# pg42819/EscTp1RayTracer

Measured on AMD Instinct MI355X. Metric: Mrays/sec + frame ms, 3840x2160 / 10k spheres, at 1/2/4/8 MI355X, higher is better.
Workload: dtype f32

## Files before the change

esctp1raytracer_amd/__init__.py:

```python
import ctypes as C

import numpy as np

from . import _capi
from ._capi import (ESC_FACE_FIXED, ESC_FACE_HASH, ESC_STAGE_AUTO, ESC_STAGE_BVH, ESC_STAGE_LDS,
                    ESC_RENDER_EXACT_ONLY, ESC_RENDER_INDEX_ORDER, ESC_RENDER_SHADE_FUSED,
                    ESC_RENDER_SHADE_QUEUE, ESC_RENDER_TIME_KERNELS, ESC_RENDER_NO_TILE_LISTS, ESC_RENDER_NO_LIGHT_LISTS, ESC_RENDER_TWO_KERNELS, ESC_RENDER_BVH_HEURISTIC_PADS, ESC_RENDER_NO_COUNTERS, ESC_RENDER_NO_PACKED_LIGHT_LISTS, ESC_RENDER_VOTE,
                    ESC_STAGE_SMEM, ESC_TRANSMIT_OFF, ESC_TRANSMIT_REFRACT, ESC_TRANSMIT_FRESNEL, EscError,
                    check)

__all__ = ["Scene", "Camera", "Renderer", "RecordedFrame", "TemporalAccumulator", "FlatScene", "MultiRenderer", "render_multi", "render_multi_rccl", "rccl_available", "strip_local_rows", "live_device_allocations", "trace", "write_ppm", "quantise", "synthetic_view", "ambient_table", "environment_sky", "environment_lookup_host",
           "EscError", "ESC_FACE_FIXED", "ESC_FACE_HASH", "ESC_STAGE_AUTO", "ESC_STAGE_SMEM",
           "ESC_STAGE_LDS", "ESC_STAGE_BVH", "ESC_RENDER_EXACT_ONLY", "ESC_RENDER_TIME_KERNELS", "ESC_RENDER_INDEX_ORDER", "ESC_RENDER_SHADE_QUEUE",
           "ESC_RENDER_SHADE_FUSED", "ESC_RENDER_NO_TILE_LISTS", "ESC_RENDER_NO_LIGHT_LISTS", "ESC_RENDER_TWO_KERNELS", "ESC_RENDER_BVH_HEURISTIC_PADS", "ESC_RENDER_NO_COUNTERS", "ESC_RENDER_NO_PACKED_LIGHT_LISTS", "ESC_RENDER_VOTE", "ESC_TRANSMIT_OFF", "ESC_TRANSMIT_REFRACT", "ESC_TRANSMIT_FRESNEL", "version"]


def _f32(a, shape=None):
    a = np.ascontiguousarray(a, dtype=np.float32)
    if shape is not None:
        a = a.reshape(shape)
    return a


def _fp(a):
# ... 970 lines not shown
                "cap": hdr[5], "global_cap": hdr[6], "counts": cnt.reshape(hdr[4], hdr[3])}

    def tile_list_ids(self, which, index):
        hdr = (C.c_int32 * 8)()
        if check(self._lib.esc_tile_list_counts(self._h, which, hdr, None, 0)) == 0:
            return np.zeros(0, np.int32), 0
        cap = hdr[6] if index < 0 else hdr[5]
        ids = np.zeros(cap, np.int32)
        n = check(self._lib.esc_tile_list_ids(self._h, which, int(index),
                                              ids.ctypes.data_as(C.POINTER(C.c_int32)), cap))
        return ids[:min(n, cap)].copy(), n

    def tile_list_global(self, which):
        return self.tile_list_ids(which, -1)

    def light_lists(self, which):
        info = (C.c_int32 * 8)()
        i32 = C.POINTER(C.c_int32)
        n = check(self._lib.esc_light_list_read(self._h, which, info, None, None, 0, 0, None))
        if n == 0:
            return None
        n_listed, R, cap, gcap = info[0], info[1], info[2], info[3]
        per_light = 6 * R * R
        face_counts = np.zeros((n_listed, 6), np.int32)
        face_ids = np.zeros((n_listed, 6, gcap), np.int32)
        ids = np.zeros((n_listed, 6, R, R, cap), np.int32)
        for li in range(n_listed):
            check(self._lib.esc_light_list_read(self._h, which, info, face_counts.ctypes.data_as(i32),
                                                face_ids.ctypes.data_as(i32), li * per_light, per_light,
                                                ids[li].ctypes.data_as(i32)))
# ... 203 lines not shown
```

esctp1raytracer_amd/_capi.py:

```python
import ctypes as C
import os

_HERE = os.path.dirname(os.path.abspath(__file__))
LIB_PATH = os.environ.get("ESC_LIB_PATH") or os.path.join(_HERE, "lib", "libesctp1rt.so")

ESC_OK = 0
ESC_ERR_INVALID = -1
ESC_ERR_HIP = -2
ESC_ERR_IO = -3
ESC_ERR_PARSE = -4
ESC_ERR_NOMEM = -5
ESC_ERR_NO_DEVICE = -6
ESC_ERR_RCCL = -7

ESC_FACE_FIXED = 0
ESC_FACE_HASH = 1
ESC_STAGE_AUTO = 0
ESC_STAGE_SMEM = 1
ESC_STAGE_LDS = 2
ESC_STAGE_BVH = 3
ESC_MATERIAL_FLOATS = 13
ESC_TRANSMISSION_FLOATS = 4
ESC_TRANSMIT_OFF = 0
ESC_TRANSMIT_REFRACT = 1
# ... 210 lines not shown
    "esc_frame_destroy": (None, [_P]),
    "esc_strip_local_rows": (C.c_int, [C.c_int32, C.c_int32, C.c_int32, C.c_int32]),
    "esc_assemble_strips": (C.c_int, [_P, _P, C.c_int32, C.c_size_t, C.c_int32, C.c_int32,
                                      C.c_int32, C.c_int32, _P]),
    "esc_build_accel": (C.c_int, [_P, _F]),
    "esc_get_accel_info": (C.c_int, [_P, C.POINTER(esc_accel_info)]),
    "esc_scene_build_accel": (C.c_int, [_P, _F, C.c_int32, C.POINTER(esc_accel_info),
                                        C.POINTER(esc_bvh_node), C.c_int64, _I32, C.c_int64, _F,
                                        C.c_int64]),
    "esc_scene_table": (C.c_int64, [_P, C.c_int32, _P, C.c_int64]),
    "esc_queue_schedule": (C.c_int, [C.c_int32, C.c_int32, _I32, C.c_int32]),
    "esc_tri_group_record": (C.c_int, [_F, C.c_int32, _F]),
    "esc_sphere_group_record": (C.c_int, [_F, C.c_int32, _F]),
    "esc_tile_list_counts": (C.c_int, [C.c_void_p, C.c_int32, _I32, _I32, C.c_size_t]),
    "esc_tile_list_ids": (C.c_int, [C.c_void_p, C.c_int32, C.c_int64, _I32, C.c_int32]),
    "esc_light_list_read": (C.c_int, [C.c_void_p, C.c_int32, _I32, _I32, _I32, C.c_int64, C.c_int64, _I32]),
    "esc_light_list_packed_read": (C.c_int, [C.c_void_p, _I32, C.c_int64, C.c_int64, _I32, _I32]),
    "esc_tile_rect": (C.c_int, [C.POINTER(esc_camera), C.c_int32, C.c_int32, _F, C.c_double, _I32]),
    "esc_tile_band": (C.c_int, [C.POINTER(esc_camera), C.c_int32, C.c_int32, C.c_int32, C.c_int32, _F,
                                C.c_double]),
    "esc_group_order": (C.c_int, [_F, C.c_int32, C.c_int32, C.c_int32, C.c_int32, _I32]),
    "esc_last_kernel_ms": (C.c_int, [_P, _F]),
    "esc_last_frame_kernel": (C.c_int, [_P]),
    "esc_frame_tripwire": (C.c_int, [_P]),
    "esc_check_inv_det_exact": (C.c_int, [_P, C.c_uint32, C.c_uint64, C.POINTER(C.c_uint64),
                                          C.POINTER(C.c_uint32)]),
    "esc_scene_shadow_origins_inside": (C.c_int, [_P, _F]),
    "esc_reset_counters": (C.c_int, [_P]),
    "esc_read_counters": (C.c_int, [_P, C.POINTER(esc_counters)]),
    "esc_intersect_rays": (C.c_int, [_P, C.c_int64, _P, _P, _P, _P, _P, _P, _P, C.c_uint32]),
# ... 99 lines not shown
```

esctp1raytracer_amd/csrc/rt_brute.h:

```cpp
#pragma once
#include <float.h>
#include <hip/hip_runtime.h>
#include <stdint.h>

#include "rt_device.h"
#include "rt_math.h"

namespace esc {

struct Hit {
  float t;
  float v;
  int32_t idx;
};


template <typename Rec, int B, typename Fetch>
DEVINL void fetch_batch(Fetch rec, int k, Rec (&r)[B]) {
#pragma unroll
  for (int i = 0; i < B; ++i) r[i] = rec(k + i);
  __builtin_amdgcn_sched_barrier(0);
}

template <typename V, int NV>
// ... 18 lines not shown
#pragma unroll
    for (int j = 0; j < NV; ++j)
#pragma unroll
      for (int c = 0; c < LN; ++c)
#pragma unroll
        for (int i = 0; i < 2; ++i) {
          Hit &hh = h[j * LN + c];
          const float de = comp(det[j][i], c), u = comp(un[j][i], c), v = comp(vn[j][i], c);
          float t2, v2;
          if (tri_candidate(de, u, v) && tri_exact(de, u, v, T[i].tnum, hh.t, t2, v2)) {
            hh.t = t2;
            hh.v = v2;
            hh.idx = idx + i;
          }
        }
  }
}

template <typename V, int NV, typename Fetch>
DEVINL void closest_tri_primary(Fetch rec, int n, int base, const V3<V> (&d)[NV],
                                Hit (&h)[NV * lanes_of<V>::n]) {
  const int n4 = n & ~3;
  if (n4) {
    DevTriP A[2], B[2];
    fetch_batch(rec, 0, A);
    for (int k = 0; k < n4; k += 4) {
      fetch_batch(rec, rec.landed(A[1].tnum, k + 2), B);
      test_tri2_primary<V, NV>(A, base + k, d, h);
      fetch_batch(rec, rec.landed(B[1].tnum, min(k + 4, n - 2)), A);
      test_tri2_primary<V, NV>(B, base + k + 2, d, h);
// ... 1383 lines not shown
```

esctp1raytracer_amd/csrc/rt_capi.cpp:

```cpp
#include <hip/hip_runtime.h>

#include <algorithm>
#include <atomic>
#include <chrono>
#include <cmath>
#include <cstdio>
#include <cstdlib>
#include <cstring>
#include <string>
#include <vector>

#include "../host/accel_build.h"
#include "../host/scene.h"
#include "../host/scene_tables.h"
#include "rt_adaptive.h"
#include "rt_ambient.h"
#include "rt_environ.h"
#include "rt_device.h"
#include "rt_devmem.h"
#include "rt_filter.h"
#include "rt_gbuffer.h"
#include "rt_query.h"
#include "rt_shade_rays.h"
#include "rt_temporal.h"
// ... 104 lines not shown
  float prepared_origin[3] = {0, 0, 0};
  esc::RayEntry *d_ray_col = nullptr, *d_ray_row = nullptr;
  size_t ray_col_cap = 0, ray_row_cap = 0;
  struct RayKey {
    float cam[9];
    int32_t W, H;
  } ray_key{};
  bool rays_valid = false;
  int32_t *d_hits = nullptr;
  size_t hits_cap = 0;
  esc::TileLists sl{}, tl{};
  size_t list_tiles_cap = 0;
  struct ListKey {
    float cam[12];
    int32_t W, H, h0, n_local_rows, strip_rows, strip_step, n_sg, n_tg;
  } list_key{};
  bool lists_valid = false;
  bool list_ids_stale = false;
  esc::LightLists ll{}, lt{};
  int ll_alloc_lights = 0;
  size_t ll_pk_steps_cap = 0;
  int32_t ll_pk_steps = -1;
  int ll_face_mode = -1, ll_fixed_face = -1;
  bool ll_valid = false;
  bool ll_complete = false;
  float sure_origin[3] = {0, 0, 0};
  bool sure_inside = false, sure_known = false;
  int last_frame_kernel = 0;
  std::vector<esc::DevLight> h_lights;
  std::vector<esc::DevTri> h_tri;
  std::vector<esc::DevSph> h_sph;
  std::vector<float> h_light_points;
// ... 642 lines not shown
  p.strip_rows = strip_rows;
  p.strip_step = strip_step;
  p.n_tri = ctx->n_tri;
  p.n_sph = ctx->n_sph;
  p.n_lights = ctx->n_lights;
  p.n_geom = ctx->n_geom;
  p.tri = ctx->d_tri;
  p.tri_p = ctx->d_tri_p;
  p.tri_n = ctx->d_tri_n;
  p.tri_face = ctx->d_tri_face;
  p.sph = ctx->d_sph;
  p.sph_p = ctx->d_sph_p;
  p.sph2 = ctx->d_sph2;
  p.sph_f = ctx->d_sph_f;
  p.sph2_f = ctx->d_sph2_f;
  {
    static const bool env_index = [] {
      const char *e = std::getenv("ESC_ORDER");
      return e && std::strcmp(e, "index") == 0;
    }();
    const bool index_order = env_index || (opts->flags & ESC_RENDER_INDEX_ORDER);
    p.sph2_ord = index_order ? nullptr : ctx->d_sph2_ord;
    p.sph2_f_ord = index_order ? nullptr : ctx->d_sph2_f_ord;
    static const bool env_nogroups = [] {
      const char *e = std::getenv("ESC_GROUPS");
      return e && std::strcmp(e, "0") == 0;
    }();
    p.sg = ctx->sg;
    p.tg = ctx->tg;
    if (index_order || env_nogroups)
      p.sg.n_grp = p.sg.n_sup = p.sg.n_hyp = p.tg.n_grp = p.tg.n_sup = p.tg.n_hyp = 0;

  }
  p.tri_f = ctx->d_tri_f;
  p.tri_pf = ctx->d_tri_pf;
  p.tri2_pf = ctx->d_tri2_pf;
  p.tri2_f = ctx->d_tri2_f;
  p.shadow_rho_max = ctx->shadow_rho_max;
  std::memcpy(p.shadow_center, ctx->shadow_center, 12);
  std::memcpy(p.scene_lo, ctx->scene_lo, 12);
  std::memcpy(p.scene_hi, ctx->scene_hi, 12);
  {
    static const bool env_off = [] {
      const char *e = std::getenv("ESC_FILTER");
      return e && std::strcmp(e, "0") == 0;
    }();
// ... 46 lines not shown
      int e = esc_launch_ray_tables(&p, ctx->d_ray_col, ctx->d_ray_row, ctx->stream);
      if (e) {
        set_error(std::string("k_prepare_ray_tables launch: ") + hipGetErrorString((hipError_t)e));
        return ESC_ERR_HIP;
      }
      ctx->ray_key = key;
      ctx->rays_valid = true;
      ctx->epoch++;
    }
  }
  {
    static const bool env_nolists = [] {
      const char *e = std::getenv("ESC_LISTS");
      return e && std::strcmp(e, "0") == 0;
    }();
    const bool want = !env_nolists && !(opts->flags & ESC_RENDER_NO_TILE_LISTS) && p.use_filter &&
                      (p.sg.n_grp > 0 || p.tg.n_grp > 0) && eff_stage != ESC_STAGE_LDS &&
                      eff_stage != ESC_STAGE_BVH && (h0 % 4) == 0;
    if (want) {
      const int tiles_x = (W + 31) / 32, tile_rows = (n_local_rows + 3) / 4;
      const size_t n_tiles = (size_t)tiles_x * tile_rows;
      const bool need_ids[2] = {p.sg.n_grp > 0, p.tg.n_grp > 0};
      const bool grow = n_tiles > ctx->list_tiles_cap || !ctx->sl.hdr;
      if (grow || (need_ids[0] && !ctx->sl.ids) || (need_ids[1] && !ctx->tl.ids)) {
        HIP_TRY(hipStreamSynchronize(ctx->stream));
        int rc;
        if (grow) {
          ctx->list_tiles_cap = 0;
          ctx->lists_valid = false;
          for (esc::TileLists *L : {&ctx->sl, &ctx->tl}) {
            if ((rc = ctx->frame.alloc(L->hdr, (size_t)esc::kTileHdrInts))) return rc;
            if ((rc = ctx->frame.alloc(L->cnt, n_tiles))) return rc;
            if ((rc = ctx->frame.release(L->ids))) return rc;
// ... 7 lines not shown
            if ((rc = ctx->frame.alloc(L->ids, ctx->list_tiles_cap * esc::kTileListCap))) return rc;
            HIP_TRY(hipMemsetAsync(L->ids, 0, ctx->list_tiles_cap * esc::kTileListCap * 4, ctx->stream));
            ctx->lists_valid = false;
          }
        }
      }
      esc_context::ListKey key;
      std::memset(&key, 0, sizeof(key));
      std::memcpy(key.cam, cam->origin, 12);
      std::memcpy(key.cam + 3, cam->lower_left_corner, 12);
      std::memcpy(key.cam + 6, cam->horizontal, 12);
      std::memcpy(key.cam + 9, cam->vertical, 12);
      key.W = W; key.H = H; key.h0 = h0; key.n_local_rows = n_local_rows;
      key.strip_rows = strip_rows; key.strip_step = strip_step;
      key.n_sg = p.sg.n_grp; key.n_tg = p.tg.n_grp;
      p.sl = ctx->sl;
      p.tl = ctx->tl;
      p.sl.tiles_x = p.tl.tiles_x = tiles_x;
      p.sl.tile_rows = p.tl.tile_rows = tile_rows;
      p.sl.enabled = p.sg.n_grp > 0;
      p.tl.enabled = p.tg.n_grp > 0;
      if (!ctx->lists_valid || std::memcmp(&key, &ctx->list_key, sizeof(key)) != 0) {
        for (const esc::TileLists *L : {&p.sl, &p.tl}) {
          HIP_TRY(hipMemsetAsync(L->hdr, 0, (size_t)esc::kTileHdrInts * 4, ctx->stream));
          HIP_TRY(hipMemsetAsync(L->cnt, 0, n_tiles * 4, ctx->stream));
          if (ctx->list_ids_stale && L->ids)
            HIP_TRY(hipMemsetAsync(L->ids, 0, ctx->list_tiles_cap * esc::kTileListCap * 4, ctx->stream));
        }
        ctx->list_ids_stale = false;
        int e = esc_launch_tile_lists(&p, ctx->stream);
        if (e) {
          set_error(std::string("k_bin_*_groups launch: ") + hipGetErrorString((hipError_t)e));
          return ESC_ERR_HIP;
        }
        ctx->list_key = key;
        ctx->lists_valid = true;
// ... 502 lines not shown
    n = (int64_t)L.n_listed * 6 * L.R * L.R;
  }
  if (index >= n) {
    set_error("esc_tile_list_ids: index out of range");
    return ESC_ERR_INVALID;
  }
  HIP_TRY(hipSetDevice(ctx->device));
  HIP_TRY(hipStreamSynchronize(ctx->stream));
  int32_t c = 0;
  HIP_TRY(hipMemcpy(&c, d_cnt + index, 4, hipMemcpyDeviceToHost));
  const int m = std::min(std::min(c, cap), capacity);
  if (m > 0) HIP_TRY(hipMemcpy(ids, d_ids + index * cap, (size_t)m * 4, hipMemcpyDeviceToHost));
  return c;
}

int esc_light_list_read(esc_context *ctx, int32_t which, int32_t info[8], int32_t *face_counts,
                        int32_t *face_ids, int64_t first_cell, int64_t n_cells, int32_t *cell_ids) {
  if (!ctx || !info || (which != 2 && which != 3) || first_cell < 0 || n_cells < 0) {
    set_error("esc_light_list_read: bad argument");
    return ESC_ERR_INVALID;
  }
  const esc::LightLists &L = which == 2 ? ctx->ll : ctx->lt;
  if (!ctx->ll_valid || !L.hdr || !L.cnt || !L.ids || (which == 2 ? ctx->sg.n_grp : ctx->tg.n_grp) == 0) return 0;
  const int n_faces = L.n_listed * 6;
  const int64_t total = (int64_t)n_faces * L.R * L.R;
  if (first_cell > total || n_cells > total - first_cell) {
    set_error("esc_light_list_read: cells out of range");
    return ESC_ERR_INVALID;
  }
  HIP_TRY(hipSetDevice(ctx->device));
// ... 2064 lines not shown
```

esctp1raytracer_amd/csrc/rt_device.h:

```cpp
#pragma once
#include <stdint.h>

namespace esc {

struct alignas(16) DevTri {
  float v0[3];
  float e1[3];
  float e2[3];
  int32_t geom;
  int32_t pad[2];
};

struct alignas(16) DevTriP {
  float e2[3];
  float e1[3];
  float tv[3];
  float qv[3];
  float tnum;
  float pad[3];
};

struct alignas(16) DevSph {
  float cx, cy, cz, r2;
};
// ... 131 lines not shown
  double fA, fH, fV;
  float kp;
  int32_t id;
  double uA, uH, uV, vA, vH, vV;
  float kpu, kpv;
  int32_t pad[2];
};
struct TileLists {
  int32_t *hdr;
  int32_t *cnt;
  int32_t *ids;
  TileEsc *esc;
  int32_t tiles_x;
  int32_t tile_rows;
  int32_t enabled;
  int32_t pad;
};

constexpr int kLightListMax = 4;
#ifndef ESC_LL_RES
#define ESC_LL_RES 128
#endif
constexpr int kLightListRes = ESC_LL_RES;
constexpr int kLightListCap = 64;
constexpr int kLightEscCap = 1024;
struct alignas(16) LightEsc {
  float nx, ny, nz, kp;
  int32_t pair, pad[3];
};
struct alignas(8) LightCell {
  int32_t offset, n_steps;
// ... 166 lines not shown
```

esctp1raytracer_amd/csrc/rt_kernels.hip:

```cpp
#include <float.h>
#include <hip/hip_runtime.h>
#include <stdint.h>

#include <algorithm>
#include <cstdlib>
#include <type_traits>

#include "rt_device.h"
#include "rt_math.h"
#include "rt_brute.h"
#include "rt_lists.h"
#include "rt_accel.h"
#include "rt_shade.h"

namespace esc {

DEVINL DevSphF sphere_filter_record(f3 oc, float cc, float r2a) {
  const float A = (fabsf(oc.x) + fabsf(oc.y)) + fabsf(oc.z);
  const float ccm = cc - ((A * A + r2a) * 0x1p-19f + 0x1p-120f);
  DevSphF F;
  F.sx = F.sy = F.sz = 0.f;
  F.w = 2.f;
  if (ccm > 0.f) {
    const float s = (sqrtf(ccm) * 0x1.fffff8p-1f - A * 0x1.2p-21f) * 0x1.fffff8p-1f;
// ... 483 lines not shown
        const SmemFetch<DevTriP> rece{p.tg.sorted_p};
        const SmemFetch<DevIdx4> reci{p.tg.orig};
        bool listed = false;
        if (p.tl.enabled)
          listed = !tile_ok ||
                   sweep_tile_list(p.tl, tile, [&](int i0, int i1, int i2, int i3) {
                     tri2_listed_primary(recf, rece, reinterpret_cast<const int32_t *>(p.tg.orig), i0, i1, dv[0], hit);
                     tri2_listed_primary(recf, rece, reinterpret_cast<const int32_t *>(p.tg.orig), i2, i3, dv[0], hit);
                   });
        if (!listed)
          closest_tri_primary_groups(
              SmemFetch<TriPF>{reinterpret_cast<const TriPF *>(p.tg.grp_pf) + p.tg.n_grp + p.tg.n_sup},
              SmemFetch<TriPF>{reinterpret_cast<const TriPF *>(p.tg.grp_pf) + p.tg.n_grp},
              SmemFetch<TriPF>{reinterpret_cast<const TriPF *>(p.tg.grp_pf)}, recp, recf, rece, reci,
              p.tg.n_hyp, dv[0], hit);
      } else {
      const int n2 = (p.use_filter && p.n_tri >= 8) ? (p.n_tri & ~3) : 0;
      closest_tri_primary_filter(SmemFetch<TriPF>{reinterpret_cast<const TriPF *>(p.tri_pf)},
                                 SmemFetch<TriF>{reinterpret_cast<const TriF *>(p.tri_f)},
                                 SmemFetch<DevTriP>{p.tri_p}, n2, 0, dv[0], hit);
      closest_tri_primary<V, NV>(SmemFetch<DevTriP>{p.tri_p + n2}, p.n_tri - n2, n2, dv, hit);
      }
    } else {
      closest_tri_primary<V, NV>(SmemFetch<DevTriP>{p.tri_p}, p.n_tri, 0, dv, hit);
    }
    if constexpr (PX == 2) {
      if (GRP && p.use_filter && p.sg.n_grp > 0) {
        const SmemFetch<SphF2> recf{reinterpret_cast<const SphF2 *>(p.sg.sorted_f)};
        const SmemFetch<DevSphP> rece{p.sg.sorted_p};
        const SmemFetch<DevIdx4> reci{p.sg.orig};
// ... 1148 lines not shown
extern "C" int esc_launch_check_inv_det(uint32_t first, uint64_t n, unsigned long long *out, hipStream_t stream) {
  if (n == 0) return 0;
  const uint64_t per_block = 256u * 256u;
  const uint64_t blocks = (n + per_block - 1) / per_block;
  hipLaunchKernelGGL(esc::k_check_inv_det, dim3((unsigned)blocks), dim3(256), 0, stream, first,
                     (unsigned long long)n, out);
  return (int)hipGetLastError();
}

extern "C" int esc_launch_tile_lists(const esc::RenderParams *p, hipStream_t stream) {
  if (p->sl.enabled && p->sg.n_grp > 0)
    hipLaunchKernelGGL(esc::k_bin_spheres, dim3(p->sg.n_grp * esc::kSphGroup / 4), dim3(256), 0, stream, *p);
  if (p->tl.enabled && p->tg.n_grp > 0) {
    hipLaunchKernelGGL(esc::k_bin_triangles, dim3(p->tg.n_grp * esc::kTriGroup / 4), dim3(256), 0, stream, *p);
    hipLaunchKernelGGL(esc::k_bin_tri_escape, dim3((unsigned)p->tl.tile_rows), dim3(256), 0, stream, *p);
  }
  return (int)hipGetLastError();
}

extern "C" int esc_launch_light_lists(const esc::RenderParams *p, hipStream_t stream) {
  const int n_rec = p->sg.n_grp * (esc::kSphGroup / 2);
  if (p->ll.enabled && p->ll.n_listed > 0 && n_rec > 0) {
    hipLaunchKernelGGL(esc::k_bin_light_pairs, dim3((n_rec + 3) / 4), dim3(256), 0, stream, *p);
    const int n_cells = p->ll.n_listed * 6 * p->ll.R * p->ll.R;
    hipLaunchKernelGGL(esc::k_sort_light_cells<false>, dim3((n_cells + 255) / 256), dim3(256), 0, stream, *p);
  }
  const int n_trec = p->tg.n_grp * (esc::kTriGroup / 2);
  if (p->lt.enabled && p->lt.n_listed > 0 && n_trec > 0) {
    hipLaunchKernelGGL(esc::k_bin_light_tri_pairs, dim3((n_trec + 3) / 4), dim3(256), 0, stream, *p);
    const int n_cells = p->lt.n_listed * 6 * p->lt.R * p->lt.R;
// ... 158 lines not shown
```

esctp1raytracer_amd/csrc/rt_lists.h:

```cpp
#pragma once
#include <hip/hip_runtime.h>
#include <stdint.h>

#include "rt_brute.h"
#include "rt_device.h"
#include "rt_math.h"
#include "rt_tile_math.h"

namespace esc {

DEVINL void list_global(const TileLists &L, int id) {
  const int slot = atomicAdd(&L.hdr[0], 1);
  if (slot < kTileGlobalCap) L.hdr[8 + slot] = id;
}

DEVINL void list_rect(const RenderParams &p, const TileLists &L, int w0, int w1, int h0, int h1, int id,
                      int lane) {
  const int tx0 = w0 >> 5, tx1 = w1 >> 5, j0 = h0 >> 2, j1 = h1 >> 2;
  if ((long long)(tx1 - tx0 + 1) * (j1 - j0 + 1) > kTileMaxSpan) {
    if (lane == 0) list_global(L, id);
    return;
  }
  const int nx = tx1 - tx0 + 1, n = nx * (j1 - j0 + 1);
  for (int k = lane; k < n; k += 64) {
    const int r4 = band_tile_row(p, j0 + k / nx);
    if (r4 < 0) continue;
    const int tile = r4 * L.tiles_x + tx0 + k % nx;
    const int slot = atomicAdd(&L.cnt[tile], 1);
    if (slot < kTileListCap) L.ids[(size_t)tile * kTileListCap + slot] = id;
  }
}

struct HullAxes {
  double nx[3], ny[3], lo[3], hi[3];
};
DEVINL void list_rect_hull(const RenderParams &p, const TileLists &L, int w0, int w1, int h0, int h1, int id,
                           int lane, const HullAxes &A) {
  const int tx0 = w0 >> 5, tx1 = w1 >> 5, j0 = h0 >> 2, j1 = h1 >> 2;
  if ((long long)(tx1 - tx0 + 1) * (j1 - j0 + 1) > kTileMaxSpan) {
    if (lane == 0) list_global(L, id);
    return;
  }
  const int nx = tx1 - tx0 + 1, n = nx * (j1 - j0 + 1);
  for (int k = lane; k < n; k += 64) {
    const int j = j0 + k / nx, tx = tx0 + k % nx;
    const int r4 = band_tile_row(p, j);
    if (r4 < 0) continue;
    const double x0 = 32.0 * tx - 1.0, x1 = 32.0 * tx + 32.0, y0 = 4.0 * j - 1.0, y1 = 4.0 * j + 4.0;
    bool outside = false;
#pragma unroll
    for (int a = 0; a < 3; ++a) {
      const double ax0 = A.nx[a] * x0, ax1 = A.nx[a] * x1, ay0 = A.ny[a] * y0, ay1 = A.ny[a] * y1;
      const double tmin = fmin(ax0, ax1) + fmin(ay0, ay1), tmax = fmax(ax0, ax1) + fmax(ay0, ay1);
      outside |= (tmax < A.lo[a]) | (tmin > A.hi[a]);
    }
    if (outside) continue;
    const int tile = r4 * L.tiles_x + tx;
    const int slot = atomicAdd(&L.cnt[tile], 1);
    if (slot < kTileListCap) L.ids[(size_t)tile * kTileListCap + slot] = id;
  }
}

__global__ void __launch_bounds__(256) k_bin_spheres(const RenderParams p) {
  const int s = blockIdx.x * 4 + (int)(threadIdx.x >> 6);
  const int lane = (int)(threadIdx.x & 63u);
  if (s >= p.sg.n_grp * kSphGroup) return;
  const DevSph S = p.sg.sorted[s];
  if (!(S.r2 >= 0.f)) return;
  const TileLists L = p.sl;
  const CamD cam = cam_frame(p);
  if (!cam.ok) {
    if (lane == 0) L.hdr[2] = 1;
    return;
  }
  const double c[3] = {(double)S.cx - cam.o[0], (double)S.cy - cam.o[1], (double)S.cz - cam.o[2]};
  const double A1 = fabs(c[0]) + fabs(c[1]) + fabs(c[2]);
  const double R = (sqrt((double)S.r2) + 0x1.2p-10 * A1) * (1.0 + 0x1p-20) + 0x1p-22 * A1 + 0x1p-60;
  int w0, w1, h0, h1;
  const int st = sphere_pixel_rect(cam, p.W, p.H, c, R, w0, w1, h0, h1);
  if (st == 2) return;
  if (st == 0) {
    if (lane == 0) list_global(L, s);
    return;
  }
  list_rect(p, L, w0, w1, h0, h1, s, lane);
}

struct TriEscape {
  bool possible;
  bool bounded;
  f3 nh;
  float beta;
  float H;
  float U, V;
};
DEVINL TriEscape tri_escape_at(const DevTri &T, float at, float slack_k, bool &pad) {
  TriEscape E;
// ... 36 lines not shown
  return E;
}
DEVINL TriEscape tri_escape(const DevTri &T, f3 o, float slack_k) {
  const f3 tv = o - ld3(T.v0);
  const float at = (fabsf(tv.x) + fabsf(tv.y)) + fabsf(tv.z);
  bool pad;
  TriEscape E = tri_escape_at(T, at, slack_k, pad);
  if (pad || !E.bounded) return E;
  const f3 n1 = cross(ld3(T.e2), ld3(T.e1));
  const float h = fabsf(dot(tv, n1)) / sqrtf(dot(n1, n1));
  E.possible = !(h > E.H * 1.01f + 0x1p-20f * at);
  return E;
}


__global__ void __launch_bounds__(256) k_bin_triangles(const RenderParams p) {
  const int k = blockIdx.x * 4 + (int)(threadIdx.x >> 6);
  const int lane = (int)(threadIdx.x & 63u);
  if (k >= p.tg.n_grp * kTriGroup) return;
  const DevTri T = p.tg.sorted[k];
  const f3 e1f = ld3(T.e1), e2f = ld3(T.e2);
  if (e1f.x == 0.f && e1f.y == 0.f && e1f.z == 0.f && e2f.x == 0.f && e2f.y == 0.f && e2f.z == 0.f)
    return;
  const TileLists L = p.tl;
  const CamD cam = cam_frame(p);
  if (!cam.ok) {
    if (lane == 0) L.hdr[2] = 1;
    return;
  }
  const double e1[3] = {e1f.x, e1f.y, e1f.z}, e2[3] = {e2f.x, e2f.y, e2f.z};
  const double v0[3] = {(double)T.v0[0] - cam.o[0], (double)T.v0[1] - cam.o[1], (double)T.v0[2] - cam.o[2]};
  double n1[3];
  cross3(e2, e1, n1);
  const double nn = sqrt(dot3(n1, n1)), l1 = sqrt(dot3(e1, e1)), l2 = sqrt(dot3(e2, e2));
  const double s3[3] = {(e1[0] + e2[0]) / 3.0, (e1[1] + e2[1]) / 3.0, (e1[2] + e2[2]) / 3.0};
  const double q1[3] = {e1[0] - s3[0], e1[1] - s3[1], e1[2] - s3[2]}, q2[3] = {e2[0] - s3[0], e2[1] - s3[1], e2[2] - s3[2]};
  const double rho = sqrt(fmax(fmax(dot3(s3, s3), dot3(q1, q1)), dot3(q2, q2)));
  const double emax = fmax(l1, l2);
  const TriEscape E = tri_escape(T, mk(p.origin[0], p.origin[1], p.origin[2]), 1.f);
  const bool sliver = !(rho > 0x1.4p-10 * emax) || !(nn > 0.0) || !(l1 > 0.0);
  if (sliver || (E.possible && !E.bounded)) {
    if (lane == 0) list_global(L, k);
    return;
  }
  double kK = 1.0;
  if (!E.possible) {
    for (int tr = 0; tr < 3; ++tr) {
      const float kc = 0.125f * (float)(1 << tr);
      const TriEscape Ec = tri_escape(T, mk(p.origin[0], p.origin[1], p.origin[2]), kc);
      if (Ec.bounded && !Ec.possible) {
        kK = (double)kc;
        break;
      }
    }
  }
  if (E.possible && lane == 0) {
    const int slot = atomicAdd(&L.hdr[1], 1);
    if (slot < kTileEscCap) {
      TileEsc X;
      const double nh[3] = {E.nh.x, E.nh.y, E.nh.z};
      double A[3], Hh[3], V[3];
      for (int j = 0; j < 3; ++j) {
        A[j] = (double)p.llc[j] - cam.o[j];
        Hh[j] = p.horizontal[j];
        V[j] = p.vertical[j];
      }
      X.fA = dot3(A, nh);
      X.fH = dot3(Hh, nh);
      X.fV = dot3(V, nh);
      X.kp = E.beta * 1.0001f + 0x1p-20f;
      X.id = k;
      const f3 tvf = mk(p.origin[0], p.origin[1], p.origin[2]) - ld3(T.v0);
// ... 1 lines not shown
      double mu[3], mv[3];
      cross3(e2, tvd, mu);
      cross3(tvd, e1, mv);
      const double lu = sqrt(dot3(mu, mu)), lv = sqrt(dot3(mv, mv));
      const double ku = (double)E.U / lu * 1.0001 + 0x1p-20, kv = (double)E.V / lv * 1.0001 + 0x1p-20;
      const bool use_u = lu > 0.0 && ku < 0.5, use_v = lv > 0.0 && kv < 0.5;
      X.uA = use_u ? dot3(A, mu) / lu : 0.0;
      X.uH = use_u ? dot3(Hh, mu) / lu : 0.0;
      X.uV = use_u ? dot3(V, mu) / lu : 0.0;
      X.kpu = use_u ? (float)(ku * (1.0 + 0x1p-20)) : 2.f;
      X.vA = use_v ? dot3(A, mv) / lv : 0.0;
      X.vH = use_v ? dot3(Hh, mv) / lv : 0.0;
      X.vV = use_v ? dot3(V, mv) / lv : 0.0;
      X.kpv = use_v ? (float)(kv * (1.0 + 0x1p-20)) : 2.f;
      X.pad[0] = X.pad[1] = 0;
      L.esc[slot] = X;
    }
  }
  const double at = (fabs(v0[0]) + fabs(v0[1]) + fabs(v0[2])) + (fabs(e1[0]) + fabs(e1[1]) + fabs(e1[2])) +
                    (fabs(e2[0]) + fabs(e2[1]) + fabs(e2[2]));
  const double slack = 0x1p-20 * at + 0x1p-60;
  const double rp = kK * rho * (1.0 + 1e-5) + slack;
  const double ea[3] = {e1[0] / l1, e1[1] / l1, e1[2] / l1};
  double eb[3];
  cross3(n1, ea, eb);
  for (int j = 0; j < 3; ++j) eb[j] /= nn;
  const int cn = lane % 12, vi = cn >> 2;
  const double sa = (cn & 1) ? rp : -rp, sb = (cn & 2) ? rp : -rp;
  double pt[3];
  for (int j = 0; j < 3; ++j)
    pt[j] = v0[j] + (vi == 1 ? e1[j] : 0.0) + (vi == 2 ? e2[j] : 0.0) + sa * ea[j] + sb * eb[j];
  double ext[4], depth = 0.0;
  const bool bounded = sphere_pixel_extent(cam, p.W, p.H, pt, slack, ext, &depth);
  const unsigned long long front = __builtin_amdgcn_ballot_w64(depth > 0.0);
  if (__builtin_amdgcn_ballot_w64(!bounded) != 0 || (front != 0 && front != ~0ull)) {
    if (lane == 0) list_global(L, k);
    return;
  }
  const bool at_clamp = !(fabs(ext[0]) < 1e9) || !(fabs(ext[1]) < 1e9) || !(fabs(ext[2]) < 1e9) || !(fabs(ext[3]) < 1e9);
  const bool rect_only = __builtin_amdgcn_ballot_w64(at_clamp) != 0;
  const double ccx = 0.5 * (ext[0] + ext[1]), ccy = 0.5 * (ext[2] + ext[3]);
  const double chx = 0.5 * (ext[1] - ext[0]), chy = 0.5 * (ext[3] - ext[2]);
  double vx[3], vy[3];
  for (int i = 0; i < 3; ++i) {
    vx[i] = 0.25 * (__shfl(ccx, 4 * i) + __shfl(ccx, 4 * i + 1) + __shfl(ccx, 4 * i + 2) + __shfl(ccx, 4 * i + 3));
    vy[i] = 0.25 * (__shfl(ccy, 4 * i) + __shfl(ccy, 4 * i + 1) + __shfl(ccy, 4 * i + 2) + __shfl(ccy, 4 * i + 3));
  }
  HullAxes HA;
  for (int a = 0; a < 3; ++a) {
    const int b = (a + 1) % 3;
    HA.nx[a] = vy[b] - vy[a];
// ... 9 lines not shown
    HA.hi[a] = hi + pad;
  }
  for (int off = 32; off > 0; off >>= 1) {
    ext[0] = fmin(ext[0], __shfl_xor(ext[0], off));
    ext[1] = fmax(ext[1], __shfl_xor(ext[1], off));
    ext[2] = fmin(ext[2], __shfl_xor(ext[2], off));
    ext[3] = fmax(ext[3], __shfl_xor(ext[3], off));
  }
  int w0, w1, h0, h1;
  if (extent_rect(ext, p.W, p.H, w0, w1, h0, h1) == 2) return;
  if (rect_only) {
    list_rect(p, L, w0, w1, h0, h1, k, lane);
    return;
  }
  list_rect_hull(p, L, w0, w1, h0, h1, k, lane, HA);
}

constexpr int kEscRowChunk = 1024;
__global__ void __launch_bounds__(256) k_bin_tri_escape(const RenderParams p) {
  __shared__ double s_pmax[kEscRowChunk];
  const TileLists L = p.tl;
  const int r4 = (int)blockIdx.x, tid = (int)threadIdx.x;
  const int n_esc = L.hdr[1];
  if (n_esc > kTileEscCap) {
    if (r4 == 0 && tid == 0) L.hdr[2] = 1;
    return;
  }
  if (n_esc == 0) return;
  const CamD cam = cam_frame(p);
  if (!cam.ok) return;
// ... 684 lines not shown
```

include/esctp1_rt.h:

```cpp
#ifndef ESCTP1_RT_H
#define ESCTP1_RT_H

#include <stddef.h>
#include <stdint.h>

#ifdef __cplusplus
extern "C" {
#endif

enum {
  ESC_OK = 0,
  ESC_ERR_INVALID = -1,
  ESC_ERR_HIP = -2,
  ESC_ERR_IO = -3,
  ESC_ERR_PARSE = -4,
  ESC_ERR_NOMEM = -5,
  ESC_ERR_NO_DEVICE = -6,
  ESC_ERR_RCCL = -7
};

const char *esc_last_error(void);
const char *esc_version(void);

typedef struct esc_scene esc_scene;
// ... 245 lines not shown

int esc_tri_group_record(const float *v0e1e2, int32_t count, float record[12]);

int esc_sphere_group_record(const float *cxyzr2, int32_t count, float record[4]);

int esc_tile_rect(const esc_camera *cam, int32_t W, int32_t H, const float centre[3], double radius,
                  int32_t rect[4]);
int esc_tile_band(const esc_camera *cam, int32_t W, int32_t H, int32_t tile_x, int32_t row,
                  const float normal[3], double kp);

int esc_tile_list_counts(esc_context *ctx, int32_t which, int32_t hdr[8], int32_t *counts,
                         size_t capacity);

int esc_tile_list_ids(esc_context *ctx, int32_t which, int64_t index, int32_t *ids, int32_t capacity);

int esc_light_list_read(esc_context *ctx, int32_t which, int32_t info[8], int32_t *face_counts,
                        int32_t *face_ids, int64_t first_cell, int64_t n_cells, int32_t *cell_ids);

int esc_light_list_packed_read(esc_context *ctx, int32_t info[8], int64_t first_cell, int64_t n_cells,
                               int32_t *steps, int32_t *slots);

int esc_group_order(const float *xyz, int32_t count, int32_t run, int32_t big, int32_t huge,
                    int32_t *order);
int esc_last_kernel_ms(esc_context *ctx, float ms[2]);
int esc_last_frame_kernel(esc_context *ctx);
int esc_frame_tripwire(esc_context *ctx);
int esc_check_inv_det_exact(esc_context *ctx, uint32_t first_bits, uint64_t n, uint64_t *mismatches,
                            uint32_t *first_mismatch);
int esc_scene_shadow_origins_inside(const esc_scene *scene, const float origin[3]);
int esc_reset_counters(esc_context *ctx);
// ... 220 lines not shown
```

Baseline: 73920.

## Bin small triangle sets into per-tile bitmasks for primary ray culling

For scenes with at most 32 ungrouped triangles, a new binning kernel builds a 32-bit per-tile mask of the triangles that can cover each 32x4 tile. Primary rays then test only the triangles set in their tile's mask plus a global mask, instead of sweeping every triangle. The existing triangle binning is templated over a list sink versus a mask sink to support this. The change adds a binning launch per frame and changes the primary-ray path only when the scene has 1-32 triangles. The workload is 10k spheres, so it likely has few or no triangles and this path may not run at all.

```diff
diff --git a/esctp1raytracer_amd/__init__.py b/esctp1raytracer_amd/__init__.py
--- a/esctp1raytracer_amd/__init__.py
+++ b/esctp1raytracer_amd/__init__.py
@@ -1008,6 +1008,16 @@
     def tile_list_global(self, which):
         return self.tile_list_ids(which, -1)
 
+    def tile_tri_masks(self):
+        info = (C.c_int32 * 8)()
+        n = check(self._lib.esc_tile_tri_masks(self._h, info, None, 0))
+        if n == 0:
+            return None
+        m = np.zeros(n, np.uint32)
+        check(self._lib.esc_tile_tri_masks(self._h, info, m.ctypes.data_as(C.POINTER(C.c_uint32)), n))
+        return {"off": info[0], "global": int(info[1]) & 0xFFFFFFFF, "tiles_x": info[2], "tile_rows": info[3],
+                "n_tri": info[4], "masks": m.reshape(info[3], info[2])}
+
     def light_lists(self, which):
         info = (C.c_int32 * 8)()
         i32 = C.POINTER(C.c_int32)
diff --git a/esctp1raytracer_amd/_capi.py b/esctp1raytracer_amd/_capi.py
--- a/esctp1raytracer_amd/_capi.py
+++ b/esctp1raytracer_amd/_capi.py
@@ -248,6 +248,7 @@
     "esc_sphere_group_record": (C.c_int, [_F, C.c_int32, _F]),
     "esc_tile_list_counts": (C.c_int, [C.c_void_p, C.c_int32, _I32, _I32, C.c_size_t]),
     "esc_tile_list_ids": (C.c_int, [C.c_void_p, C.c_int32, C.c_int64, _I32, C.c_int32]),
+    "esc_tile_tri_masks": (C.c_int, [C.c_void_p, _I32, C.POINTER(C.c_uint32), C.c_size_t]),
     "esc_light_list_read": (C.c_int, [C.c_void_p, C.c_int32, _I32, _I32, _I32, C.c_int64, C.c_int64, _I32]),
     "esc_light_list_packed_read": (C.c_int, [C.c_void_p, _I32, C.c_int64, C.c_int64, _I32, _I32]),
     "esc_tile_rect": (C.c_int, [C.POINTER(esc_camera), C.c_int32, C.c_int32, _F, C.c_double, _I32]),
diff --git a/esctp1raytracer_amd/csrc/rt_brute.h b/esctp1raytracer_amd/csrc/rt_brute.h
--- a/esctp1raytracer_amd/csrc/rt_brute.h
+++ b/esctp1raytracer_amd/csrc/rt_brute.h
@@ -56,6 +56,37 @@
             hh.idx = idx + i;
           }
         }
+  }
+}
+
+template <typename V, int NV>
+DEVINL void test_tri_primary(const DevTriP &T, int idx, const V3<V> (&d)[NV], Hit (&h)[NV * lanes_of<V>::n]) {
+  constexpr int LN = lanes_of<V>::n;
+  V det[NV], un[NV], vn[NV];
+  bool any = false;
+#pragma unroll
+  for (int j = 0; j < NV; ++j) {
+    const V3<V> pv = cross_vu(d[j], ld3(T.e2));
+    det[j] = dotu(ld3(T.e1), pv);
+    un[j] = dotu(ld3(T.tv), pv);
+    vn[j] = dotu(ld3(T.qv), d[j]);
+#pragma unroll
+    for (int c = 0; c < LN; ++c) any |= tri_candidate(comp(det[j], c), comp(un[j], c), comp(vn[j], c));
+  }
+  if (ANY_LANE_RARE(any)) {
+#pragma unroll
+    for (int j = 0; j < NV; ++j)
+#pragma unroll
+      for (int c = 0; c < LN; ++c) {
+        Hit &hh = h[j * LN + c];
+        const float de = comp(det[j], c), u = comp(un[j], c), v = comp(vn[j], c);
+        float t2, v2;
+        if (tri_candidate(de, u, v) && tri_exact(de, u, v, T.tnum, hh.t, t2, v2)) {
+          hh.t = t2;
+          hh.v = v2;
+          hh.idx = idx;
+        }
+      }
   }
 }
 
diff --git a/esctp1raytracer_amd/csrc/rt_capi.cpp b/esctp1raytracer_amd/csrc/rt_capi.cpp
--- a/esctp1raytracer_amd/csrc/rt_capi.cpp
+++ b/esctp1raytracer_amd/csrc/rt_capi.cpp
@@ -142,8 +142,10 @@
   struct ListKey {
     float cam[12];
     int32_t W, H, h0, n_local_rows, strip_rows, strip_step, n_sg, n_tg;
+    int32_t n_mask_tri;
   } list_key{};
   bool lists_valid = false;
+  bool tri_masks_last = false;
   bool list_ids_stale = false;
   esc::LightLists ll{}, lt{};
   int ll_alloc_lights = 0;
@@ -816,6 +818,7 @@
   p.sph2 = ctx->d_sph2;
   p.sph_f = ctx->d_sph_f;
   p.sph2_f = ctx->d_sph2_f;
+  bool linear_sweeps = false;
   {
     static const bool env_index = [] {
       const char *e = std::getenv("ESC_ORDER");
@@ -832,6 +835,7 @@
     p.tg = ctx->tg;
     if (index_order || env_nogroups)
       p.sg.n_grp = p.sg.n_sup = p.sg.n_hyp = p.tg.n_grp = p.tg.n_sup = p.tg.n_hyp = 0;
+    linear_sweeps = index_order || env_nogroups;
 
   }
   p.tri_f = ctx->d_tri_f;
@@ -908,9 +912,12 @@
       const char *e = std::getenv("ESC_LISTS");
       return e && std::strcmp(e, "0") == 0;
     }();
-    const bool want = !env_nolists && !(opts->flags & ESC_RENDER_NO_TILE_LISTS) && p.use_filter &&
-                      (p.sg.n_grp > 0 || p.tg.n_grp > 0) && eff_stage != ESC_STAGE_LDS &&
-                      eff_stage != ESC_STAGE_BVH && (h0 % 4) == 0;
+    const bool allowed = !env_nolists && !(opts->flags & ESC_RENDER_NO_TILE_LISTS) && p.use_filter &&
+                         eff_stage != ESC_STAGE_LDS && eff_stage != ESC_STAGE_BVH && (h0 % 4) == 0;
+    const bool px2 = opts->pixels_per_lane == 0 || opts->pixels_per_lane == 2;
+    const bool want_masks = allowed && px2 && !linear_sweeps && p.n_tri > 0 && p.n_tri <= 32;
+    const bool want = allowed && (p.sg.n_grp > 0 || p.tg.n_grp > 0 || want_masks);
+    ctx->tri_masks_last = want_masks;
     if (want) {
       const int tiles_x = (W + 31) / 32, tile_rows = (n_local_rows + 3) / 4;
       const size_t n_tiles = (size_t)tiles_x * tile_rows;
@@ -948,12 +955,15 @@
       key.W = W; key.H = H; key.h0 = h0; key.n_local_rows = n_local_rows;
       key.strip_rows = strip_rows; key.strip_step = strip_step;
       key.n_sg = p.sg.n_grp; key.n_tg = p.tg.n_grp;
+      key.n_mask_tri = want_masks ? p.n_tri : 0;
       p.sl = ctx->sl;
       p.tl = ctx->tl;
       p.sl.tiles_x = p.tl.tiles_x = tiles_x;
       p.sl.tile_rows = p.tl.tile_rows = tile_rows;
       p.sl.enabled = p.sg.n_grp > 0;
       p.tl.enabled = p.tg.n_grp > 0;
+      p.sl.masks = 0;
+      p.tl.masks = want_masks ? 1 : 0;
       if (!ctx->lists_valid || std::memcmp(&key, &ctx->list_key, sizeof(key)) != 0) {
         for (const esc::TileLists *L : {&p.sl, &p.tl}) {
           HIP_TRY(hipMemsetAsync(L->hdr, 0, (size_t)esc::kTileHdrInts * 4, ctx->stream));
@@ -1486,6 +1496,25 @@
   return c;
 }
 
+int esc_tile_tri_masks(esc_context *ctx, int32_t info[8], uint32_t *masks, size_t capacity) {
+  if (!ctx || !info) {
+    set_error("esc_tile_tri_masks: bad argument");
+    return ESC_ERR_INVALID;
+  }
+  const esc::TileLists &L = ctx->tl;
+  if (!ctx->tri_masks_last || !ctx->lists_valid || !L.hdr || !L.cnt || ctx->list_key.n_mask_tri <= 0) return 0;
+  HIP_TRY(hipSetDevice(ctx->device));
+  HIP_TRY(hipStreamSynchronize(ctx->stream));
+  int32_t h[5];
+  HIP_TRY(hipMemcpy(h, L.hdr, sizeof(h), hipMemcpyDeviceToHost));
+  const int tiles_x = (ctx->list_key.W + 31) / 32, tile_rows = (ctx->list_key.n_local_rows + 3) / 4;
+  const int32_t out[8] = {h[2], h[4], tiles_x, tile_rows, ctx->list_key.n_mask_tri, 0, 0, 0};
+  std::memcpy(info, out, sizeof(out));
+  const size_t n_tiles = (size_t)tiles_x * tile_rows;
+  if (masks) HIP_TRY(hipMemcpy(masks, L.cnt, std::min(capacity, n_tiles) * 4, hipMemcpyDeviceToHost));
+  return (int)n_tiles;
+}
+
 int esc_light_list_read(esc_context *ctx, int32_t which, int32_t info[8], int32_t *face_counts,
                         int32_t *face_ids, int64_t first_cell, int64_t n_cells, int32_t *cell_ids) {
   if (!ctx || !info || (which != 2 && which != 3) || first_cell < 0 || n_cells < 0) {
diff --git a/esctp1raytracer_amd/csrc/rt_device.h b/esctp1raytracer_amd/csrc/rt_device.h
--- a/esctp1raytracer_amd/csrc/rt_device.h
+++ b/esctp1raytracer_amd/csrc/rt_device.h
@@ -169,7 +169,7 @@
   int32_t tiles_x;
   int32_t tile_rows;
   int32_t enabled;
-  int32_t pad;
+  int32_t masks;
 };
 
 constexpr int kLightListMax = 4;
diff --git a/esctp1raytracer_amd/csrc/rt_kernels.hip b/esctp1raytracer_amd/csrc/rt_kernels.hip
--- a/esctp1raytracer_amd/csrc/rt_kernels.hip
+++ b/esctp1raytracer_amd/csrc/rt_kernels.hip
@@ -521,6 +521,16 @@
               SmemFetch<TriPF>{reinterpret_cast<const TriPF *>(p.tg.grp_pf) + p.tg.n_grp},
               SmemFetch<TriPF>{reinterpret_cast<const TriPF *>(p.tg.grp_pf)}, recp, recf, rece, reci,
               p.tg.n_hyp, dv[0], hit);
+      } else if (p.tl.masks && ((ListPtr)(uintptr_t)p.tl.hdr)[2] == 0) {
+        uint32_t m = 0;
+        if (tile_ok)
+          m = (uint32_t)(((ListPtr)(uintptr_t)p.tl.cnt)[tile] | ((ListPtr)(uintptr_t)p.tl.hdr)[4]);
+        const SmemFetch<DevTriP> rec{p.tri_p};
+        while (m) {
+          const int k = __builtin_ctz(m);
+          m &= m - 1;
+          test_tri_primary<V, NV>(rec(k), k, dv, hit);
+        }
       } else {
       const int n2 = (p.use_filter && p.n_tri >= 8) ? (p.n_tri & ~3) : 0;
       closest_tri_primary_filter(SmemFetch<TriPF>{reinterpret_cast<const TriPF *>(p.tri_pf)},
@@ -1699,6 +1709,12 @@
   if (p->tl.enabled && p->tg.n_grp > 0) {
     hipLaunchKernelGGL(esc::k_bin_triangles, dim3(p->tg.n_grp * esc::kTriGroup / 4), dim3(256), 0, stream, *p);
     hipLaunchKernelGGL(esc::k_bin_tri_escape, dim3((unsigned)p->tl.tile_rows), dim3(256), 0, stream, *p);
+  }
+  if (p->tl.masks && p->n_tri > 0 && p->n_tri <= 32) {
+    const long long n_tiles = (long long)p->tl.tiles_x * p->tl.tile_rows;
+    const long long want = n_tiles / (256 * 16);
+    const unsigned parts = (unsigned)(want < 1 ? 1 : want > 64 ? 64 : want);
+    hipLaunchKernelGGL(esc::k_bin_tri_masks, dim3((unsigned)p->n_tri, parts), dim3(256), 0, stream, *p);
   }
   return (int)hipGetLastError();
 }
diff --git a/esctp1raytracer_amd/csrc/rt_lists.h b/esctp1raytracer_amd/csrc/rt_lists.h
--- a/esctp1raytracer_amd/csrc/rt_lists.h
+++ b/esctp1raytracer_amd/csrc/rt_lists.h
@@ -9,40 +9,62 @@
 
 namespace esc {
 
-DEVINL void list_global(const TileLists &L, int id) {
-  const int slot = atomicAdd(&L.hdr[0], 1);
-  if (slot < kTileGlobalCap) L.hdr[8 + slot] = id;
-}
-
-DEVINL void list_rect(const RenderParams &p, const TileLists &L, int w0, int w1, int h0, int h1, int id,
-                      int lane) {
+struct TileListSink {
+  TileLists L;
+  static constexpr bool kEscEntries = true;
+  static constexpr long long kMaxSpan = kTileMaxSpan;
+  DEVINL int part() const { return 0; }
+  DEVINL int parts() const { return 1; }
+  DEVINL void off() const { L.hdr[2] = 1; }
+  DEVINL void global(int id) const {
+    const int slot = atomicAdd(&L.hdr[0], 1);
+    if (slot < kTileGlobalCap) L.hdr[8 + slot] = id;
+  }
+  DEVINL void tile(int tile, int id) const {
+    const int slot = atomicAdd(&L.cnt[tile], 1);
+    if (slot < kTileListCap) L.ids[(size_t)tile * kTileListCap + slot] = id;
+  }
+};
+struct TileMaskSink {
+  TileLists L;
+  int part_, parts_;
+  static constexpr bool kEscEntries = false;
+  static constexpr long long kMaxSpan = 0x7fffffffll;
+  DEVINL int part() const { return part_; }
+  DEVINL int parts() const { return parts_; }
+  DEVINL void off() const { L.hdr[2] = 1; }
+  DEVINL void global(int id) const { atomicOr(&L.hdr[4], (int)(1u << id)); }
+  DEVINL void tile(int tile, int id) const { atomicOr(&L.cnt[tile], (int)(1u << id)); }
+};
+
+template <typename Sink>
+DEVINL void list_rect(const RenderParams &p, const Sink &S, int w0, int w1, int h0, int h1, int id, int lane) {
   const int tx0 = w0 >> 5, tx1 = w1 >> 5, j0 = h0 >> 2, j1 = h1 >> 2;
-  if ((long long)(tx1 - tx0 + 1) * (j1 - j0 + 1) > kTileMaxSpan) {
-    if (lane == 0) list_global(L, id);
+  if ((long long)(tx1 - tx0 + 1) * (j1 - j0 + 1) > Sink::kMaxSpan) {
+    if (lane == 0) S.global(id);
     return;
   }
   const int nx = tx1 - tx0 + 1, n = nx * (j1 - j0 + 1);
-  for (int k = lane; k < n; k += 64) {
+  for (int k = lane + 64 * S.part(); k < n; k += 64 * S.parts()) {
     const int r4 = band_tile_row(p, j0 + k / nx);
     if (r4 < 0) continue;
-    const int tile = r4 * L.tiles_x + tx0 + k % nx;
-    const int slot = atomicAdd(&L.cnt[tile], 1);
-    if (slot < kTileListCap) L.ids[(size_t)tile * kTileListCap + slot] = id;
+    S.tile(r4 * S.L.tiles_x + tx0 + k % nx, id);
   }
 }
 
 struct HullAxes {
   double nx[3], ny[3], lo[3], hi[3];
 };
-DEVINL void list_rect_hull(const RenderParams &p, const TileLists &L, int w0, int w1, int h0, int h1, int id,
+template <typename Sink>
+DEVINL void list_rect_hull(const RenderParams &p, const Sink &S, int w0, int w1, int h0, int h1, int id,
                            int lane, const HullAxes &A) {
   const int tx0 = w0 >> 5, tx1 = w1 >> 5, j0 = h0 >> 2, j1 = h1 >> 2;
-  if ((long long)(tx1 - tx0 + 1) * (j1 - j0 + 1) > kTileMaxSpan) {
-    if (lane == 0) list_global(L, id);
+  if ((long long)(tx1 - tx0 + 1) * (j1 - j0 + 1) > Sink::kMaxSpan) {
+    if (lane == 0) S.global(id);
     return;
   }
   const int nx = tx1 - tx0 + 1, n = nx * (j1 - j0 + 1);
-  for (int k = lane; k < n; k += 64) {
+  for (int k = lane + 64 * S.part(); k < n; k += 64 * S.parts()) {
     const int j = j0 + k / nx, tx = tx0 + k % nx;
     const int r4 = band_tile_row(p, j);
     if (r4 < 0) continue;
@@ -55,9 +77,7 @@
       outside |= (tmax < A.lo[a]) | (tmin > A.hi[a]);
     }
     if (outside) continue;
-    const int tile = r4 * L.tiles_x + tx;
-    const int slot = atomicAdd(&L.cnt[tile], 1);
-    if (slot < kTileListCap) L.ids[(size_t)tile * kTileListCap + slot] = id;
+    S.tile(r4 * S.L.tiles_x + tx, id);
   }
 }
 
@@ -67,10 +87,10 @@
   if (s >= p.sg.n_grp * kSphGroup) return;
   const DevSph S = p.sg.sorted[s];
   if (!(S.r2 >= 0.f)) return;
-  const TileLists L = p.sl;
+  const TileListSink L{p.sl};
   const CamD cam = cam_frame(p);
   if (!cam.ok) {
-    if (lane == 0) L.hdr[2] = 1;
+    if (lane == 0) L.off();
     return;
   }
   const double c[3] = {(double)S.cx - cam.o[0], (double)S.cy - cam.o[1], (double)S.cz - cam.o[2]};
@@ -80,7 +100,7 @@
   const int st = sphere_pixel_rect(cam, p.W, p.H, c, R, w0, w1, h0, h1);
   if (st == 2) return;
   if (st == 0) {
-    if (lane == 0) list_global(L, s);
+    if (lane == 0) L.global(s);
     return;
   }
   list_rect(p, L, w0, w1, h0, h1, s, lane);
@@ -147,18 +167,13 @@
 }
 
 
-__global__ void __launch_bounds__(256) k_bin_triangles(const RenderParams p) {
-  const int k = blockIdx.x * 4 + (int)(threadIdx.x >> 6);
-  const int lane = (int)(threadIdx.x & 63u);
-  if (k >= p.tg.n_grp * kTriGroup) return;
-  const DevTri T = p.tg.sorted[k];
+template <typename Sink> DEVINL void bin_triangle(const RenderParams &p, const DevTri &T, int k, int lane, const Sink &L) {
   const f3 e1f = ld3(T.e1), e2f = ld3(T.e2);
   if (e1f.x == 0.f && e1f.y == 0.f && e1f.z == 0.f && e2f.x == 0.f && e2f.y == 0.f && e2f.z == 0.f)
     return;
-  const TileLists L = p.tl;
   const CamD cam = cam_frame(p);
   if (!cam.ok) {
-    if (lane == 0) L.hdr[2] = 1;
+    if (lane == 0) L.off();
     return;
   }
   const double e1[3] = {e1f.x, e1f.y, e1f.z}, e2[3] = {e2f.x, e2f.y, e2f.z};
@@ -172,8 +187,8 @@
   const double emax = fmax(l1, l2);
   const TriEscape E = tri_escape(T, mk(p.origin[0], p.origin[1], p.origin[2]), 1.f);
   const bool sliver = !(rho > 0x1.4p-10 * emax) || !(nn > 0.0) || !(l1 > 0.0);
-  if (sliver || (E.possible && !E.bounded)) {
-    if (lane == 0) list_global(L, k);
+  if (sliver || (E.possible && (!E.bounded || !Sink::kEscEntries))) {
+    if (lane == 0) L.global(k);
     return;
   }
   double kK = 1.0;
@@ -187,8 +202,8 @@
       }
     }
   }
-  if (E.possible && lane == 0) {
-    const int slot = atomicAdd(&L.hdr[1], 1);
+  if (Sink::kEscEntries && E.possible && lane == 0) {
+    const int slot = atomicAdd(&L.L.hdr[1], 1);
     if (slot < kTileEscCap) {
       TileEsc X;
       const double nh[3] = {E.nh.x, E.nh.y, E.nh.z};
@@ -220,7 +235,7 @@
       X.vV = use_v ? dot3(V, mv) / lv : 0.0;
       X.kpv = use_v ? (float)(kv * (1.0 + 0x1p-20)) : 2.f;
       X.pad[0] = X.pad[1] = 0;
-      L.esc[slot] = X;
+      L.L.esc[slot] = X;
     }
   }
   const double at = (fabs(v0[0]) + fabs(v0[1]) + fabs(v0[2])) + (fabs(e1[0]) + fabs(e1[1]) + fabs(e1[2])) +
@@ -240,7 +255,7 @@
   const bool bounded = sphere_pixel_extent(cam, p.W, p.H, pt, slack, ext, &depth);
   const unsigned long long front = __builtin_amdgcn_ballot_w64(depth > 0.0);
   if (__builtin_amdgcn_ballot_w64(!bounded) != 0 || (front != 0 && front != ~0ull)) {
-    if (lane == 0) list_global(L, k);
+    if (lane == 0) L.global(k);
     return;
   }
   const bool at_clamp = !(fabs(ext[0]) < 1e9) || !(fabs(ext[1]) < 1e9) || !(fabs(ext[2]) < 1e9) || !(fabs(ext[3]) < 1e9);
@@ -280,6 +295,21 @@
     return;
   }
   list_rect_hull(p, L, w0, w1, h0, h1, k, lane, HA);
+}
+
+__global__ void __launch_bounds__(256) k_bin_triangles(const RenderParams p) {
+  const int k = blockIdx.x * 4 + (int)(threadIdx.x >> 6);
+  const int lane = (int)(threadIdx.x & 63u);
+  if (k >= p.tg.n_grp * kTriGroup) return;
+  bin_triangle(p, p.tg.sorted[k], k, lane, TileListSink{p.tl});
+}
+
+__global__ void __launch_bounds__(256) k_bin_tri_masks(const RenderParams p) {
+  const int k = (int)blockIdx.x;
+  const int lane = (int)(threadIdx.x & 63u);
+  if (k >= p.n_tri || k >= 32) return;
+  const TileMaskSink S{p.tl, (int)(blockIdx.y * 4 + (threadIdx.x >> 6)), (int)gridDim.y * 4};
+  bin_triangle(p, p.tri[k], k, lane, S);
 }
 
 constexpr int kEscRowChunk = 1024;
diff --git a/include/esctp1_rt.h b/include/esctp1_rt.h
--- a/include/esctp1_rt.h
+++ b/include/esctp1_rt.h
@@ -283,6 +283,8 @@
 
 int esc_tile_list_ids(esc_context *ctx, int32_t which, int64_t index, int32_t *ids, int32_t capacity);
 
+int esc_tile_tri_masks(esc_context *ctx, int32_t info[8], uint32_t *masks, size_t capacity);
+
 int esc_light_list_read(esc_context *ctx, int32_t which, int32_t info[8], int32_t *face_counts,
                         int32_t *face_ids, int64_t first_cell, int64_t n_cells, int32_t *cell_ids);
 
```

Result: faster. 77460, median of 6 (+4.8%).
